# leducthanhig/image-restoration-models

Measured on AMD Instinct MI355X. Metric: images/sec + PSNR, Restormer motion-deblur 1280x720, higher is better.
Workload: dtype f32 (1x1 convs: fp32 emulated by 3 fp16 MFMAs on hi/lo operand splits with fp32 accumulation, error vs float64 at the level of an fp32 chain; everything else exact f32; value_exact_f32: f32 MFMA everywhere); 1 GPU; Restormer motion-deblur (WithBias LN, 26.13M params, synthetic weights seed 42) on 1280x720x3 uint8 GoPro-shaped synthetic frames; 6 tiles 512x512 (overlap 96) per frame; a step = 4 frame(s) per GPU, their 24 tiles in one batched forward; global_batch=4, tile=512, overlap=96, parallelism=per-image shard x1, no data-path collective

## Files before the change

### image-restoration-models_amd/_hip.py

```python
from __future__ import annotations

import ctypes as C
import os

import torch

_HERE = os.path.dirname(os.path.abspath(__file__))
LIB_PATH = os.path.join(_HERE, "libirm_hip.so")

ACT_NONE, ACT_RELU, ACT_GELU, ACT_SILU, ACT_RELU6 = 0, 1, 2, 3, 4
LN_NONE, LN_WITHBIAS, LN_BIASFREE = 0, 1, 2

_P, _L, _I, _F, _D = C.c_void_p, C.c_long, C.c_int, C.c_float, C.c_double

SIGNATURES = {
    "irm_version": [],
    "irm_ln_stats_f32": [_P, _L, _P, _I, _I, _I, _F, _P],
    "irm_gemm1x1_f32": [_P, _L, _P, _L, _P, _L, _P, _L, _P, _P, _P, _P, _I, _I, _I, _I, _I, _I, _I, _I, _P, _F, _P, _P],
    "irm_gemm1x1_f16x3_f32": [_P, _L, _P, _L, _P, _L, _P, _L, _P, _P, _P, _P, _I, _I, _I, _I, _I, _I, _I, _I, _P, _F, _P, _P],
    "irm_ln_split_f16": [_P, _L, _P, _P, _I, _F, _F, _P, _I, _I, _I, _P],
    "irm_ln_gemm_presplit_f16x3_f32": [_P, _P, _L, _P, _P, _I, _F, _F, _P, _L, _P, _F, _I, _I, _I, _I, _I, _P],
    "irm_ln_gemm_presplit_cl_f16x3_f32": [_P, _P, _L, _P, _P, _I, _F, _F, _P, _L, _P, _F, _I, _I, _I, _I, _I, _I, _P],
    "irm_gdfn_tail_f16x3_f32": [_P, _L, _P, _P, _P, _P, _L, _F, _I, _I, _I, _I, _I, _I, _P],
    "irm_gemm_presplit_f16x3_f32": [_P, _P, _P, _L, _P, _F, _I, _I, _I, _I, _I, _I, _I, _I, _P],
# ... 21 lines not shown
    "irm_conv3x3_f16x3_ep_f32": [_P, _F, _P, _L, _P, _L, _P, _L, _P, _I, _I, _I, _I, _I, _I, _F, _I, _I, _I, _I, _I, _I, _P],
    "irm_tile_extract": [_P, _I, _P, _P, _P, _I, _I, _I, _I, _I, _I, _I, _I, _F, _F, _I, _P],
    "irm_chan_stats_f32": [_P, _L, _P, _I, _I, _I, _F, _P],
    "irm_chan_stats_ws_f32": [_P, _L, _P, _P, _L, _I, _I, _I, _F, _P],
    "irm_chan_norm_act_f32": [_P, _L, _P, _P, _P, _P, _L, _P, _L, _I, _I, _I, _I, _P],
    "irm_conv3x3_s2_f32": [_P, _L, _P, _P, _L, _I, _I, _I, _I, _I, _P],
    "irm_dwconv3x3_s2_f32": [_P, _L, _P, _P, _L, _I, _I, _I, _I, _P],
    "irm_upsample_add_f32": [_P, _L, _P, _L, _P, _L, _I, _I, _I, _I, _I, _P],
    "irm_transpose_f32": [_P, _L, _P, _L, _I, _I, _I, _P],
    "irm_selective_scan_f32": [_P, _P, _P, _P, _P, _P, _P, _P, _P, _P, _P, _I, _I, _I, _I, _I, _I, _P],
    "irm_losh_combine_f32": [_P, _P, _P, _P, _P, _P, _P, _P, _L, _P, _L, _I, _I, _I, _I, _F, _P],
    "irm_window_blend": [_P, _P, _P, _P, _I, _P, _P, _I, _I, _I, _I, _I, _I, _I, _I, _I, _I, _F, _F, _P],
    "irm_window_blend_scaled": [_P, _P, _P, _P, _I, _P, _P, _I, _I, _I, _I, _I, _I, _I, _I, _I, _I, _I, _F, _F, _P],
    "irm_frame_metrics": [_P, _P, _I, _I, _I, _I, _I, _D, _P, _P, _P, _L, _P],
    "irm_imresize_bicubic": [_P, _I, _P, _I, _P, _P, _P, _P, _I, _I, _I, _I, _I, _I, _P],
    "irm_frame_metrics_basicsr": [_P, _P, _I, _I, _I, _I, _I, _I, _I, _I, _P, _P, _P, _L, _P],
    "irm_niqe_features": [_P, _I, _I, _I, _I, _I, _I, _I, _P, _P, _P, _L, _P],
    "irm_dihedral_chop_f32": [_P, _P, _P, _L, _I, _I, _I, _I, _I, _I, _I, _P],
    "irm_ensemble_merge_f32": [_P, _P, _P, _L, _I, _I, _I, _I, _I, _I, _P],
}

SIGNATURES_HALF = {
    "irm_conv3x3_h_in_f32": [_P, _P, _L, _P, _L, _P, _I, _I, _I, _I, _I, _I, _P],
    "irm_conv3x3_h_f16": [_P, _F, _P, _L, _P, _L, _P, _L, _P, _I, _I, _I, _I, _I, _I, _I, _I, _P],
    "irm_conv3x3_h_out_f32": [_P, _P, _L, _P, _L, _P, _L, _P, _I, _I, _I, _I, _I, _I, _P],
}

SIGNATURES_FRAMES = {
    "irm_frame_minmax_f32": [_P, _L, _P, _P, _L, _P],
    "irm_tile_extract_f32": [_P, _P, _P, _P, _P, _I, _I, _I, _I, _I, _I, _I, _I, _I, _P],
    "irm_window_blend_f32": [_P, _P, _P, _P, _P, _I, _I, _I, _I, _I, _I, _I, _I, _I, _I, _I, _P],
}

_lib = None


class HipLibraryError(RuntimeError):
    pass


def load():
    global _lib, LIB_PATH
    if _lib is None:
        if os.environ.get("IRM_HIP_LIB"):
            LIB_PATH = os.path.abspath(os.environ["IRM_HIP_LIB"])
        if not os.path.exists(LIB_PATH):
            raise HipLibraryError(
                f"{LIB_PATH} not found: build it with `python -c 'import __graft_entry__ as g; g.build()'` "
                "(make -C image-restoration-models_amd/csrc).  There is no CPU fallback.")
        lib = C.CDLL(LIB_PATH)
        for name, argtypes in {**SIGNATURES, **SIGNATURES_HALF, **SIGNATURES_FRAMES}.items():
            fn = getattr(lib, name)
            fn.argtypes = argtypes
            fn.restype = _I
        _lib = lib
    return _lib


def _stream() -> int:
    return torch.cuda.current_stream().cuda_stream


def ptr(t):
    if t is None:
        return None
    if isinstance(t, int):
        return t
    assert t.is_cuda, "HIP kernels need device tensors"
    return t.data_ptr()


def call(name: str, *args):
    rc = getattr(load(), name)(*args, _stream())
    if rc != 0:
        raise HipLibraryError(f"{name} failed with status {rc} "
                              f"({'invalid arguments' if rc == -1 else 'HIP launch error'})")



def pack_gemm_weight(w: torch.Tensor) -> torch.Tensor:
    w = w.detach().reshape(w.shape[0], -1).float()
    m, k = w.shape
    mt, ks = (m + 15) // 16, 4 * ((k + 15) // 16)
    wpad = torch.zeros(mt * 16, ks * 4, dtype=torch.float32, device=w.device)
# ... 402 lines not shown
```

### image-restoration-models_amd/csrc/fused_qkv_cm.hip

```cpp
#include "irm_common.h"

#define QC_TH 8
#define QC_TW 32
#define QC_PITCH 36
#define QC_SLOTS ((QC_TH + 2) * QC_PITCH)
#define QC_PT 23
#define QC_CS 1728
#define QC_IMG (32 * QC_CS)

struct QcArgs {
    const float* X; long x_bs;
    float* Y; long y_bs;
    const float* rec;
    int C, H, W, S, M;
    int ln_mode; float eps, inv_s1;
    int x_tm, v_tm;
    int tiles_x, tiles, items, gpx;
    const float* gscale;
    float* part;
};
#define QC_NCH 4

__device__ __forceinline__ unsigned qc_row(int c) {
    const int i = c & 15;
    const int rk = i < 4 ? i : i < 12 ? i - 4 : i - 8;
    const int o = (rk >> 1) * 4 + (rk & 1);
    const int fix = (16 - ((c * (QC_CS / 16)) & 15)) & 15;
    return (unsigned)(c * QC_CS + 16 * ((o + fix) & 15));
}

template <int KS, bool GRAM = false>
__global__ __launch_bounds__(512, 2) void qkv_cm_kernel(QcArgs a) {
    static_assert(!GRAM || KS == 2, "GRAM: C = 48");
    constexpr int W1F = KS * 1024, RECF = W1F + 512, RECP = KS * 4 + 2;
    constexpr int SLOT_B = RECF * 4, CF_OFF = W1F * 4;
    constexpr int OSC_OFF = 3 * SLOT_B, MSK_OFF = OSC_OFF + 368 * 4, PL_OFF = MSK_OFF + 368 * 4;
    static_assert(PL_OFF % 16 == 0 && PL_OFF + 2 * QC_IMG <= 160 * 1024, "LDS");
    static_assert(15 * 16 + 368 * 4 <= QC_CS, "row + phase shift inside the row stride");
    extern __shared__ __attribute__((aligned(16))) float smem[];
    irm_lc* lds = (irm_lc*)smem;
    float* slots = smem;

    const int wave = __builtin_amdgcn_readfirstlane((int)threadIdx.x >> 6);
    const long plane = (long)a.H * a.W;
    const int S = a.S;
    const int per = GRAM ? (a.items / QC_NCH + 7) >> 3 : (a.items + 7) >> 3;
    const int xcd = blockIdx.x & 7, pos = blockIdx.x >> 3;
    auto item_of = [&](int round) {
        if constexpr (GRAM) {
            const int i = (round / QC_NCH) * a.gpx + pos;
            return i < per ? (xcd * per + i) * QC_NCH + round % QC_NCH : a.items;
        }
        const int i = round * a.gpx + pos; return i < per ? xcd * per + i : a.items;
    };

    int round = 0;
    int item = item_of(0);
    if (item >= a.items) return;
    float xr[3][KS][8];
    f32x4 gacc[GRAM ? 3 : 1][GRAM ? 3 : 1];
    float gnq[3] = {0.f, 0.f, 0.f}, gnk[3] = {0.f, 0.f, 0.f};
    if constexpr (GRAM) {
#pragma unroll
        for (int x = 0; x < 3; ++x)
#pragma unroll
            for (int y = 0; y < 3; ++y) gacc[x][y] = (f32x4){0.f, 0.f, 0.f, 0.f};
    }
    for (;;) {
        int tid = threadIdx.x;
        asm volatile("" : "+v"(tid));
        const int lane = tid & 63, g = lane >> 4, r = lane & 15;
        const int b = item / a.tiles, tile = item - b * a.tiles;
        const int ty0 = (tile / a.tiles_x) * QC_TH, tx0 = (tile % a.tiles_x) * QC_TW;
        float* Y = a.Y + (long)b * a.y_bs;
        const int nitem = item_of(round + 1);
        const unsigned vw = irm_opaque((unsigned)(lane * 16));

        bool inside[3];
#pragma unroll
        for (int j = 0; j < 3; ++j) {
            const int p = 16 * (wave + 8 * j) + r, ph = p / QC_PITCH, pc = p - ph * QC_PITCH;
            const int gy0 = ty0 - 1 + ph, gx0 = tx0 - 1 + pc;
            inside[j] = p < QC_SLOTS && pc < QC_TW + 2 && gy0 >= 0 && gy0 < a.H && gx0 >= 0 && gx0 < a.W;
        }
        auto load_x = [&](int item) {
            int t2 = threadIdx.x;
            asm volatile("" : "+v"(t2));
            const int r = t2 & 15, g = (t2 & 63) >> 4;
            const int b = item / a.tiles, tile = item - b * a.tiles;
            const int ty0 = (tile / a.tiles_x) * QC_TH, tx0 = (tile % a.tiles_x) * QC_TW;
            const float* X = a.X + (long)b * a.x_bs;
#pragma unroll
        for (int j = 0; j < 3; ++j) {
            const int p = 16 * (wave + 8 * j) + r, ph = p / QC_PITCH, pc = p - ph * QC_PITCH;
            const int gy0 = ty0 - 1 + ph, gx0 = tx0 - 1 + pc;
            const int gy = min(max(gy0, 0), a.H - 1), gx = min(max(gx0, 0), a.W - 1);
            if (a.x_tm) {
                const float* xp = X + (unsigned)((((gy >> 3) * a.tiles_x + (gx >> 5)) * 256 + (gy & 7) * QC_TW + (gx & 31)) * a.C);
#pragma unroll
                for (int ks = 0; ks < KS; ++ks) {
// ... 105 lines not shown
                        acc[j] = __builtin_amdgcn_mfma_f32_16x16x32_f16(xl[j][ks], bh, acc[j], 0, 0, 0);
                        acc[j] = __builtin_amdgcn_mfma_f32_16x16x32_f16(xh[j][ks], bh, acc[j], 0, 0, 0);
                    }
                }
                const float b1 = irm_ld<float>(lds, (unsigned)(r * 4), slot * SLOT_B + CF_OFF + 320 * 4 + hct * 64);
                const unsigned vr = hct ? vrow1 : vrow0;
#pragma unroll
                for (int j = 0; j < 3; ++j) {
                    if (wave + 8 * j < QC_PT) {
                        f32x4 h;
#pragma unroll
                        for (int e = 0; e < 4; ++e) h[e] = fmaf(acc[j][e], osc4[j][e], b1 * msk4[j][e]);
                        irm_st<f32x4>(lds, vr + (unsigned)((16 * (wave + 8 * j) + 4 * g) * 4), PL_OFF + img * QC_IMG, h);
                    }
                }
            }
        };
        auto gemm1 = [&](int slot, int img) { gemm1h(slot, img, 0); gemm1h(slot, img, 1); };
        f32x4 sp0[3], sp1[3];
        irm_v2 sp2[3];
        float stap[10];
        auto st_read = [&](int slot, int img, int hct) {
            const unsigned vr = (hct ? vrow1 : vrow0) + (unsigned)((wave * QC_PITCH + 8 * g) * 4);
            const unsigned vt = (unsigned)((16 * hct + r) * 4);
#pragma unroll
            for (int dy = 0; dy < 3; ++dy) {
                sp0[dy] = irm_ld<f32x4>(lds, vr, PL_OFF + img * QC_IMG + dy * QC_PITCH * 4);
                sp1[dy] = irm_ld<f32x4>(lds, vr, PL_OFF + img * QC_IMG + dy * QC_PITCH * 4 + 16);
                sp2[dy] = irm_ld<irm_v2>(lds, vr, PL_OFF + img * QC_IMG + dy * QC_PITCH * 4 + 32);
            }
#pragma unroll
            for (int t = 0; t < 10; ++t) stap[t] = irm_ld<float>(lds, vt, slot * SLOT_B + CF_OFF + t * 128);
        };
        irm_h8 gqh[GRAM ? 3 : 1], gql[GRAM ? 3 : 1];
        auto st_comp = [&](int st, int hct, auto UC) {
            {
                constexpr int U = decltype(UC)::value;
                const int ch = 32 * st + 16 * hct + r;
                float o[8];
#pragma unroll
                for (int e = 0; e < 8; ++e) o[e] = stap[9];
#pragma unroll
                for (int dy = 0; dy < 3; ++dy) {
                    const float P[10] = {sp0[dy][0], sp0[dy][1], sp0[dy][2], sp0[dy][3], sp1[dy][0], sp1[dy][1], sp1[dy][2], sp1[dy][3],
                                         sp2[dy][0], sp2[dy][1]};
#pragma unroll
                    for (int dx = 0; dx < 3; ++dx) {
                        const float t = stap[dy * 3 + dx];
#pragma unroll
                        for (int e = 0; e < 8; ++e) o[e] = fmaf(t, P[e + dx], o[e]);
                    }
                }
                if constexpr (GRAM && U >= 0 && U < 6) {
                    const float sc = a.gscale[16 * U + r];
                    float nn = 0.f, xs[8];
#pragma unroll
                    for (int e = 0; e < 8; ++e) { nn = fmaf(o[e], o[e], nn); xs[e] = o[e] * sc; }
                    irm_h8 hi, lo;
                    irm_split8(xs, hi, lo);
                    if constexpr (U < 3) {
                        gnq[U] += nn; gqh[U] = hi; gql[U] = lo;
                    } else {
                        gnk[U - 3] += nn;
#pragma unroll
                        for (int x = 0; x < 3; ++x) {
                            f32x4& t = gacc[x][U - 3];
                            t = irm_mfma3_f16(gqh[x], gql[x], hi, lo, t);
                        }
                    }
                    return;
                }
                if (ch >= a.M) return;
                if (ch < 2 * a.C) {
                    float* yt = Y + (long)tile * (2L * a.C * 256) + ch * 256 + wave * QC_TW + 8 * g;
                    *reinterpret_cast<f32x4*>(yt) = (f32x4){o[0], o[1], o[2], o[3]};
                    *reinterpret_cast<f32x4*>(yt + 4) = (f32x4){o[4], o[5], o[6], o[7]};
                } else if (a.v_tm) {
                    float* yt = Y + 2L * a.C * plane + (long)tile * (a.C * 256L) + (wave * QC_TW + 8 * g) * a.C + (ch - 2 * a.C);
#pragma unroll
                    for (int e = 0; e < 8; ++e) yt[e * a.C] = o[e];
                } else {
                    float* yt = Y + (long)ch * plane + (long)(ty0 + wave) * a.W + tx0 + 8 * g;
                    *reinterpret_cast<f32x4*>(yt) = (f32x4){o[0], o[1], o[2], o[3]};
                    *reinterpret_cast<f32x4*>(yt + 4) = (f32x4){o[4], o[5], o[6], o[7]};
                }
            }
        };

        gemm1(0, 0);
        asm volatile("s_waitcnt lgkmcnt(0)" ::: "memory");
        __builtin_amdgcn_s_barrier();
        constexpr std::integral_constant<int, -1> NOU{};
        if constexpr (GRAM) {
            irm_for<5>([&](auto ITC) {
                constexpr int it = decltype(ITC)::value;
                constexpr int s1c = (it + 1) % 3, s3c = it % 3;
                if constexpr (it + 1 < 5) {
                    if constexpr (it + 3 <= 5) irm_dma<RECP>(a.rec + (long)(it + 3) * RECF, slots + s3c * RECF, wave, lane);
                    st_read(s1c, it & 1, 0); gemm1h(s1c, (it + 1) & 1, 0); st_comp(it, 0, std::integral_constant<int, 2 * it>{});
                    st_read(s1c, it & 1, 1); gemm1h(s1c, (it + 1) & 1, 1); st_comp(it, 1, std::integral_constant<int, 2 * it + 1>{});
                    if constexpr (it + 3 <= 5) asm volatile("s_waitcnt vmcnt(0) lgkmcnt(0)" ::: "memory");
                    else asm volatile("s_waitcnt lgkmcnt(0)" ::: "memory");
// ... 4 lines not shown
                    asm volatile("s_waitcnt lgkmcnt(0)" ::: "memory");
                }
                __builtin_amdgcn_s_barrier();
            });
        } else {
        const int it_pf = max(S - 3, 0);
        int s1 = 1, s3 = 0;
        for (int it = 0; it + 1 < S; ++it) {
            const bool dma = it + 3 <= S;
            if (dma) irm_dma<RECP>(a.rec + (long)(it + 3) * RECF, slots + s3 * RECF, wave, lane);
            st_read(s1, it & 1, 0); gemm1h(s1, (it + 1) & 1, 0); st_comp(it, 0, NOU);
            st_read(s1, it & 1, 1); gemm1h(s1, (it + 1) & 1, 1); st_comp(it, 1, NOU);
            if (it <= it_pf) asm volatile("s_waitcnt vmcnt(0) lgkmcnt(0)" ::: "memory");
            else asm volatile("s_waitcnt lgkmcnt(0)" ::: "memory");
            if (PREFETCH && it == it_pf) { load_x(min(nitem, a.items - 1)); __builtin_amdgcn_sched_barrier(0); }
            __builtin_amdgcn_s_barrier();
            s1 = s1 == 2 ? 0 : s1 + 1;
            s3 = s3 == 2 ? 0 : s3 + 1;
        }
        {
            const int it = S - 1;
            if (!PREFETCH || S < 2) {
                load_x(min(nitem, a.items - 1));
                __builtin_amdgcn_sched_barrier(0);
            }
            st_read(s1, it & 1, 0); st_comp(it, 0, NOU);
            st_read(s1, it & 1, 1); st_comp(it, 1, NOU);
            asm volatile("s_waitcnt lgkmcnt(0)" ::: "memory");
            __builtin_amdgcn_s_barrier();
        }
        }
        if constexpr (GRAM) {
            if (round % QC_NCH == QC_NCH - 1) {
                constexpr int REC = 48 * 48 + 96;
#pragma unroll
                for (int t = 0; t < 3; ++t) {
                    gnq[t] += __shfl_xor(gnq[t], 16); gnq[t] += __shfl_xor(gnq[t], 32);
                    gnk[t] += __shfl_xor(gnk[t], 16); gnk[t] += __shfl_xor(gnk[t], 32);
                }
                float* mine = reinterpret_cast<float*>(smem) + PL_OFF / 4 + wave * REC;
                float isk[3];
#pragma unroll
                for (int y = 0; y < 3; ++y) isk[y] = 1.0f / a.gscale[48 + 16 * y + r];
#pragma unroll
                for (int x = 0; x < 3; ++x) {
                    const f32x4 sq4 = *reinterpret_cast<const f32x4*>(a.gscale + 16 * x + 4 * g);
#pragma unroll
                    for (int e = 0; e < 4; ++e) {
                        const float isq = 1.0f / sq4[e];
#pragma unroll
                        for (int y = 0; y < 3; ++y) mine[(16 * x + 4 * g + e) * 48 + 16 * y + r] = gacc[x][y][e] * (isq * isk[y]);
                    }
                    if (g == 0) { mine[48 * 48 + 16 * x + r] = gnq[x]; mine[48 * 48 + 48 + 16 * x + r] = gnk[x]; }
                }
                __syncthreads();
                const float* all = reinterpret_cast<const float*>(smem) + PL_OFF / 4;
                float* out = a.part + ((long)b * (a.tiles / QC_NCH) + tile / QC_NCH) * REC;
                for (int e = threadIdx.x; e < REC; e += 512) {
                    float sum = all[e];
#pragma unroll
                    for (int w = 1; w < 8; ++w) sum += all[w * REC + e];
                    out[e] = sum;
                }
#pragma unroll
                for (int x = 0; x < 3; ++x) {
                    gnq[x] = 0.f; gnk[x] = 0.f;
#pragma unroll
                    for (int y = 0; y < 3; ++y) gacc[x][y] = (f32x4){0.f, 0.f, 0.f, 0.f};
                }
            }
        }
        if (nitem >= a.items) break;
        item = nitem;
        ++round;
    }
}

template <int KS, bool GRAM = false>
static int qc_launch(QcArgs a, int B, hipStream_t stream) {
    const size_t lds = (size_t)3 * (KS * 1024 + 512) * 4 + 2 * 368 * 4 + 2 * QC_IMG;
    IRM_ALLOW_BIG_LDS((&qkv_cm_kernel<KS, GRAM>));
    int dev = 0, n = 0;
    if (hipGetDevice(&dev) != hipSuccess ||
        hipDeviceGetAttribute(&n, hipDeviceAttributeMultiprocessorCount, dev) != hipSuccess || n <= 0) return IRM_ELAUNCH;
    a.tiles_x = a.W / QC_TW;
    a.tiles = a.tiles_x * (a.H / QC_TH);
    a.items = B * a.tiles;
    const int per = GRAM ? (a.items / QC_NCH + 7) >> 3 : (a.items + 7) >> 3;
    a.gpx = (n + 7) / 8;
    if (a.gpx > per) a.gpx = per;
    hipLaunchKernelGGL((qkv_cm_kernel<KS, GRAM>), dim3(a.gpx * 8), dim3(512), lds, stream, a);
    return irm_launch_status();
}

extern "C" int irm_qkv_gram_cm_f16x3_f32(const float* rec, const float* x, long x_bs, float* y, long y_bs, const float* gscale,
                                         float* part, int ln_mode, float eps, float inv_s1, int B, int C, int H, int W, int x_tm,
                                         int v_tm, hipStream_t stream) {
    if (!rec || !x || !y || !gscale || !part || x == y || B <= 0 || H <= 0 || W <= 0) return IRM_EINVAL;
    if (C != 48 || (H & 7) || (W & 31) || ((H / 8) * (W / 32)) % QC_NCH || (long)3 * C * H * W >= (1L << 30)) return IRM_EINVAL;
    if (ln_mode != IRM_LN_WITHBIAS && ln_mode != IRM_LN_BIASFREE) return IRM_EINVAL;
    if ((x_bs & 3) || (y_bs & 3) || !irm_aligned16(x) || !irm_aligned16(y) || !irm_aligned16(rec) || !irm_aligned16(gscale)) return IRM_EINVAL;
    QcArgs a;
// ... 24 lines not shown
```

### image-restoration-models_amd/ops.py

```python
from __future__ import annotations

import os

import torch

from . import _hip
from ._hip import ACT_GELU, ACT_NONE, ACT_RELU, ACT_RELU6, ACT_SILU, LN_BIASFREE, LN_NONE, LN_WITHBIAS


class KernelTimer:

    def __init__(self, detail=False, only=None):
        self.records = []
        self.detail = detail
        self.only = None if only is None else frozenset(only)
        self._chain = {}
        self._done = {}
        self._since = 0

    def _fold(self, k, e0, e1, fl, by):
        d = self._done.setdefault(k, dict(launches=0, ms=0.0, flops=0.0, bytes=0.0))
        d["launches"] += 1
        d["ms"] += e0.elapsed_time(e1)
        d["flops"] += fl
# ... 285 lines not shown
    rec = c * c + 2 * c
    if c in (48, 96) and N % 64 == 0:
        slots, best = 2 * 256, None
        for chunk in range(128, 4096 + 1, 64):
            nchunk = -(-N // chunk)
            cost = -(-(B * heads * nchunk) // slots) * (chunk + 192)
            if best is None or cost < best[0]:
                best = (cost, chunk, nchunk)
        return best[1], best[2], rec
    nsub = (c // (16 * sb)) ** 2
    chunk = -(-(N * B * heads * nsub) // (4 * target_blocks()))
    chunk = min(max(-(-chunk // 64) * 64, 256), 4096)
    return chunk, -(-N // chunk), rec


QKV_GRAM_NCH = 4


def can_qkv_gram(C: int, heads: int, H: int, W: int) -> bool:
    return C == 48 and heads == 1 and H % 8 == 0 and W % 32 == 0 and ((H // 8) * (W // 32)) % QKV_GRAM_NCH == 0


def qkv_gram_cm(pk, x, y, gram_scale, part, C: int, *, ln_mode, eps: float = 1e-5, x_tm: bool = False, v_tm: bool = False) -> int:
    _chk(x, "x"), _chk(y, "y")
    B, _, H, W = x.shape
    assert can_qkv_gram(C, 1, H, W) and y.shape[1] == 3 * C and gram_scale.numel() == 2 * C
    rec, inv_s1 = pk
    N = H * W
    nchunk = (H // 8) * (W // 32) // QKV_GRAM_NCH
    assert part.numel() >= B * nchunk * (C * C + 2 * C)
    _launch("qkv_dw_fused", B * N * (2.0 * 3 * C * C + 18.0 * 3 * C + 2.0 * C * C), 4.0 * B * N * 2 * C, "irm_qkv_gram_cm_f16x3_f32",
            _hip.ptr(rec), _hip.ptr(x), _bs(x), _hip.ptr(y), _bs(y), _hip.ptr(gram_scale), _hip.ptr(part), int(ln_mode),
            float(eps), float(inv_s1), B, C, H, W, int(x_tm), int(v_tm), tag=f"C{C} {H}x{W} B{B} gram")
    return nchunk


def mdta_fold(qkv, part, gsum, temperature, wout, mfold, C: int, heads: int, attn=None, split: bool = False,
              gram_scale=None, frag: bool = False, tm: bool = False, nchunk_ready: int | None = None):
    _chk(qkv, "qkv")
    B, _, H, W = qkv.shape
    N = H * W
    chunk, nchunk, rec = mdta_plan(B, C, heads, N)
    if nchunk_ready is not None:
        nchunk = nchunk_ready
    assert part.numel() >= B * heads * nchunk * rec and gsum.numel() >= B * heads * rec
    c = C // heads
    assert not tm or (c in (48, 96) and N % 256 == 0), "tile-major q, k: the LDS-DMA ring passes only"
    if nchunk_ready is not None:
        pass
    elif gram_scale is not None and c in (48, 96) and N % 64 == 0:
        assert gram_scale.numel() == 2 * C and gram_scale.is_contiguous()
        _launch("mdta_gram_f16x3", 2.0 * B * heads * c * c * N, 8.0 * B * C * N,
                "irm_mdta_gram_tm_f16x3_f32" if tm else "irm_mdta_gram_f16x3_f32", _hip.ptr(qkv),
                _bs(qkv), _hip.ptr(gram_scale), _hip.ptr(part), B, C, heads, N, chunk,
                tag=f"C{C} h{heads} N{N} B{B} chunk{chunk}")
    else:
        _launch("mdta_gram", 2.0 * B * heads * c * c * N, 8.0 * B * C * N, "irm_mdta_gram_tm_f32" if tm else "irm_mdta_gram_f32",
                _hip.ptr(qkv), _bs(qkv), _hip.ptr(part), B, C, heads, N, chunk, tag=f"C{C} h{heads} N{N} B{B} chunk{chunk}")
    _launch("mdta_finalize", 2.0 * B * C * C * c, 4.0 * B * (heads * nchunk * rec + C * C),
            "irm_mdta_finalize_frag_f16x3_f32" if frag else "irm_mdta_finalize_f16x3_f32" if split else "irm_mdta_finalize_f32",
            _hip.ptr(part), _hip.ptr(gsum), _hip.ptr(temperature), _hip.ptr(wout), _hip.ptr(mfold), _hip.ptr(attn),
            B, C, heads, nchunk, tag=f"C{C} h{heads} nchunk{nchunk} B{B}")


def can_fuse_stats(M: int) -> bool:
    mt = (M + 15) // 16
# ... 154 lines not shown
```

### image-restoration-models_amd/restormer/restormer.py

```python
from __future__ import annotations

import os

import torch
import torch.nn as nn

from .. import _hip, ops

SYNTH_RULES = (
    (r"^output\.weight$", "gain", 0.02),
    (r"^skip_conv\.weight$", "gain", 0.5),
)


def _hidden(dim, factor):
    return int(dim * factor)


class _Norm(nn.Module):

    def __init__(self, dim, kind):
        super().__init__()
        self.body = nn.Module()
        self.body.weight = nn.Parameter(torch.ones(dim))
# ... 119 lines not shown
                a, ff = m.attn, m.ffn
                pk[name] = dict(
                    qkv=_hip.pack_gemm_weight(a.qkv.weight), qkv_b=f32(a.qkv.bias),
                    qkv_dw=f32(a.qkv_dwconv.weight.reshape(-1, 9)), qkv_dw_b=f32(a.qkv_dwconv.bias),
                    wout=f32(a.project_out.weight.reshape(m.dim, m.dim)), wout_b=f32(a.project_out.bias),
                    temp=f32(a.temperature.reshape(-1)),
                    pin=_hip.pack_gemm_weight(ff.project_in.weight), pin_b=f32(ff.project_in.bias),
                    ffn_dw=f32(ff.dwconv.weight.reshape(-1, 9)), ffn_dw_b=f32(ff.dwconv.bias),
                    pout=_hip.pack_gemm_weight(ff.project_out.weight), pout_b=f32(ff.project_out.bias),
                    n1w=f32(m.norm1.w), n1b=f32(m.norm1.b), n2w=f32(m.norm2.w), n2b=f32(m.norm2.b))
                if self._split:
                    if _hip.split_is_safe(a.qkv.weight, m.norm1.w, m.norm1.b):
                        pk[name]["qkv_s"] = _hip.pack_gemm_weight_split(a.qkv.weight)
                    if _hip.split_is_safe(ff.project_in.weight, m.norm2.w, m.norm2.b):
                        pk[name]["pin_s"] = _hip.pack_gemm_weight_split(ff.project_in.weight)
                    if _hip.split_is_safe(ff.project_out.weight):
                        pk[name]["pout_s"] = _hip.pack_gemm_weight_split(ff.project_out.weight)
                    pk[name]["mfold_split"] = _hip.split_is_safe(a.project_out.weight)
                    if m.dim == 192:
                        hp = 64 * -(-ff.hidden // 64)
                        frag, s_w, bp = _hip.pack_pin_padded(ff.project_in.weight, ff.project_in.bias, hp)
                        s_x = _hip.ln_split_scale(m.norm2.w, m.norm2.b, m.dim, m.norm2.mode == ops.LN_WITHBIAS)
                        pk[name]["pin_cl"] = (frag, 1.0 / (s_w * s_x), s_x, bp, hp)
                        pk[name]["tail"] = _hip.pack_gdfn_tail(ff.dwconv.weight, ff.dwconv.bias, ff.project_out.weight)
                    if m.dim in (192, 384):
                        for slot, conv, nrm in (("qkv_ps", a.qkv, m.norm1), ("pin_ps", ff.project_in, m.norm2)):
                            frag, s_w = _hip.pack_gemm_weight_presplit(conv.weight)
                            s_x = _hip.ln_split_scale(nrm.w, nrm.b, m.dim, nrm.mode == ops.LN_WITHBIAS)
                            pk[name][slot] = (frag, 1.0 / (s_w * s_x), s_x)
                    gs = _hip.gram_scales(a.qkv.weight, a.qkv.bias, a.qkv_dwconv.weight, a.qkv_dwconv.bias, m.norm1.w,
                                          m.norm1.b, m.norm1.mode == ops.LN_WITHBIAS)
                    if gs is not None:
                        pk[name]["gram_s"] = gs.to(a.qkv.weight.device)
                if self._split and ops.can_fuse_gdfn(m.dim, 4):
                    pk[name].update(
                        qkv_f=_hip.pack_qkv_fused(a.qkv.weight, a.qkv.bias, a.qkv_dwconv.weight, a.qkv_dwconv.bias,
                                                  m.norm1.w, m.norm1.b),
                        gdfn_f=_hip.pack_gdfn_fused(ff.project_in.weight, ff.project_in.bias, ff.dwconv.weight,
                                                    ff.dwconv.bias, ff.project_out.weight, m.norm2.w, m.norm2.b))
                    if pk[name]["mfold_split"] and m.dim % 16 == 0:
                        pk[name]["gdfn_fa"] = _hip.pack_gdfn_fused(
                            ff.project_in.weight, ff.project_in.bias, ff.dwconv.weight, ff.dwconv.bias,
                            ff.project_out.weight, m.norm2.w, m.norm2.b, kperm=True)
                if ops.can_fuse_dw(m.dim, 4):
                    c, dw, dwb = m.dim, a.qkv_dwconv.weight.reshape(-1, 9), a.qkv_dwconv.bias
                    pk[name].update(
                        v_dwp=_hip.pack_dw_table(dw[2 * c:], None if dwb is None else dwb[2 * c:], c, False),
                        ffn_dwp=_hip.pack_dw_table(ff.dwconv.weight, ff.dwconv.bias, ff.hidden, True))
        for name in ("down1_2", "down2_3", "down3_4", "up4_3", "up3_2", "up2_1"):
            pk[name] = _hip.pack_conv3x3(getattr(self, name).body[0].weight)
        pk["patch_embed"] = _hip.pack_conv3x3(self.patch_embed.proj.weight)
        pk["patch_embed_b"] = f32(self.patch_embed.proj.bias)
        pk["output"] = _hip.pack_conv3x3(self.output.weight)
        pk["output_b"] = f32(self.output.bias)
        for name in ("reduce_chan_level3", "reduce_chan_level2") + (("skip_conv",) if self.dual_pixel_task else ()):
            pk[name] = _hip.pack_gemm_weight(getattr(self, name).weight)
            pk[name + "_b"] = f32(getattr(self, name).bias)
            if self._split and name != "skip_conv" and _hip.split_is_safe(getattr(self, name).weight):
                pk[name + "_s"] = _hip.pack_gemm_weight_split(getattr(self, name).weight)
        self._packed, self._packed_key = pk, key
        return pk

    @property
    def _ws(self):
        return self._ws_by_stream.setdefault(torch.cuda.current_stream().cuda_stream if torch.cuda.is_available()
                                             else 0, {})
# ... 15 lines not shown
        return t

    def release_workspace(self):
        self._ws_by_stream.clear()

    def _block(self, blk: TransformerBlock, w: dict, x: torch.Tensor, have_stats: bool = False,
               want_stats: bool = True) -> bool:
        B, C, H, W = x.shape
        N = H * W
        dev = x.device
        heads = blk.attn.num_heads
        hid = blk.ffn.hidden
        fuse = ops.can_fuse_stats(C)
        stats = self._buf("stats", B * 2 * N, dev)
        big_a = self._buf("scratch_a", B * max(3 * C, 2 * hid) * N, dev)
        big_b = self._buf("scratch_b", B * max(3 * C, hid) * N, dev)
        qkv = big_a[:B * 3 * C * N].view(B, 3 * C, H, W)
        qkv2 = big_b[:B * 3 * C * N].view(B, 3 * C, H, W)
        split = self._split and N % 4 == 0
        s_qkv, s_pin, s_pout = split and "qkv_s" in w, split and "pin_s" in w, split and "pout_s" in w
        s_fold = split and w.get("mfold_split", False)
        presplit = split and "qkv_ps" in w and ops.can_presplit(C, N)
        if presplit:
            xs = self._buf("xsplit", B * C * N, dev)
            frag, out_scale, s_x = w["qkv_ps"]
            ops.ln_gemm_presplit(frag, x, qkv, 3 * C, C, w["n1w"], w["n1b"], blk.norm1.mode, s_x, out_scale=out_scale,
                                 bias=w["qkv_b"], xs=xs)
        else:
            if not have_stats:
                ops.ln_stats(x, stats)
            ops.gemm1x1(w["qkv_s" if s_qkv else "qkv"], x, qkv, 3 * C, C, bias=w["qkv_b"], stats=stats, lnw=w["n1w"],
                        lnb=w["n1b"], ln_mode=blk.norm1.mode, split=s_qkv)
        fuse_dw = "v_dwp" in w and ops.can_fuse_dw(C, W)
        if fuse_dw:
            ops.dwconv3x3(qkv[:, :2 * C], w["qkv_dw"], qkv2[:, :2 * C],
                          bias=None if w["qkv_dw_b"] is None else w["qkv_dw_b"][:2 * C])
        else:
            ops.dwconv3x3(qkv, w["qkv_dw"], qkv2, bias=w["qkv_dw_b"])
        _, nchunk, rec = ops.mdta_plan(B, C, heads, N)
        part = self._buf("gram_part", B * heads * nchunk * rec, dev)
        gsum = self._buf("gram_sum", B * heads * rec, dev)
        mfold_n = ops.mfold_numel(C)
        mfold = self._zeros(("mfold", C, B), B * mfold_n, dev)
        ops.mdta_fold(qkv2, part, gsum, w["temp"], w["wout"], mfold, C, heads, split=s_fold,
                      gram_scale=w.get("gram_s") if split else None)
        if fuse_dw:
            ops.dwgemm(mfold, w["v_dwp"], qkv[:, 2 * C:], x, C, C, gate=False, res=x, bias=w["wout_b"],
                       w_bs=mfold_n, stats_out=stats if fuse else None, split=s_fold)
        else:
            ops.gemm1x1(mfold, qkv2[:, 2 * C:], x, C, C, res=x, bias=w["wout_b"], w_bs=mfold_n,
                        stats_out=stats if fuse else None, split=s_fold)
        if split and "tail" in w and ops.can_gdfn_tail(C, H, W):
            frag, out_scale, s_x, bp, hp = w["pin_cl"]
            h_cl = self._buf("h_cl", B * 2 * hp * N, dev)
            ops.ln_gemm_presplit_cl(frag, x, h_cl, 2 * hp, C, w["n2w"], w["n2b"], blk.norm2.mode, s_x, out_scale=out_scale, bias=bp)
            ops.gdfn_tail(w["tail"], h_cl, x, C, hid, hp, bias=w["pout_b"])
            return False
        h = big_a[:B * 2 * hid * N].view(B, 2 * hid, H, W)
        g = big_b[:B * hid * N].view(B, hid, H, W)
        if presplit:
            frag, out_scale, s_x = w["pin_ps"]
            ops.ln_gemm_presplit(frag, x, h, 2 * hid, C, w["n2w"], w["n2b"], blk.norm2.mode, s_x, out_scale=out_scale,
                                 bias=w["pin_b"], xs=xs)
        else:
            if not fuse:
                ops.ln_stats(x, stats)
            ops.gemm1x1(w["pin_s" if s_pin else "pin"], x, h, 2 * hid, C, bias=w["pin_b"], stats=stats, lnw=w["n2w"],
                        lnb=w["n2b"], ln_mode=blk.norm2.mode, split=s_pin)
        emit = fuse and want_stats
        if fuse_dw:
            ops.dwgemm(w["pout_s" if s_pout else "pout"], w["ffn_dwp"], h, x, C, hid, gate=True, res=x,
                       bias=w["pout_b"], stats_out=stats if emit else None, split=s_pout)
        else:
            ops.dwconv3x3_gate(h, w["ffn_dw"], g, bias=w["ffn_dw_b"])
            ops.gemm1x1(w["pout_s" if s_pout else "pout"], g, x, C, hid, res=x, bias=w["pout_b"],
                        stats_out=stats if emit else None, split=s_pout)
        return emit

# ... 127 lines not shown
```

### include/irm_hip.h

```cpp
#ifndef IRM_HIP_H
#define IRM_HIP_H

#ifdef __cplusplus
extern "C" {
#endif

typedef struct ihipStream_t* irm_stream_t;

#define IRM_OK 0
#define IRM_EINVAL (-1)
#define IRM_ELAUNCH (-2)

#define IRM_ACT_NONE 0
#define IRM_ACT_RELU 1
#define IRM_ACT_GELU 2
#define IRM_ACT_SILU 3

#define IRM_LN_NONE 0
#define IRM_LN_WITHBIAS 1
#define IRM_LN_BIASFREE 2

int irm_version(void);

int irm_ln_stats_f32(const float* x, long x_bs, float* stats, int B, int C, int N, float eps,
// ... 124 lines not shown
int irm_chan_stats_f32(const float* x, long x_bs, float* stats, int B, int C, int N, float eps, irm_stream_t stream);
int irm_chan_stats_ws_f32(const float* x, long x_bs, float* stats, float* ws, long ws_floats, int B, int C, int N,
                          float eps, irm_stream_t stream);
int irm_chan_norm_act_f32(const float* x, long x_bs, const float* stats, const float* w, const float* b,
                          const float* res, long r_bs, float* y, long y_bs, int B, int C, int N, int act,
                          irm_stream_t stream);
int irm_conv3x3_s2_f32(const float* x, long x_bs, const float* w, float* y, long y_bs, int B, int Ci, int Co, int H,
                       int W, irm_stream_t stream);
int irm_dwconv3x3_s2_f32(const float* x, long x_bs, const float* w, float* y, long y_bs, int B, int C, int H, int W,
                         irm_stream_t stream);
int irm_upsample_add_f32(const float* src, long s_bs, const float* add, long a_bs, float* out, long o_bs, int B, int C,
                         int Hs, int Ws, int scale, irm_stream_t stream);

int irm_dihedral_chop_f32(const float* src, const int* table, float* dst, long dst_pixels, int B, int C, int H, int W,
                          int P, int max_ph, int max_pw, irm_stream_t stream);
int irm_ensemble_merge_f32(const float* pred, const int* table, float* out, long pred_pixels, int B, int Co, int H,
                           int W, int P, int scale, irm_stream_t stream);

int irm_transpose_f32(const float* in, long in_bs, float* out, long out_bs, int B, int R, int C,
                      irm_stream_t stream);

int irm_selective_scan_f32(const float* xT, const float* pT, const int* ids, const float* dtw, const float* dtb,
                           const float* A, const float* Dskip, float* yT, float* state, float* sdt, float* ysum,
                           int B, int L, int D, int N, int R, int chunk, irm_stream_t stream);

int irm_losh_combine_f32(float* ysum, const float* gw, const float* gb, float* gate, const float* yT,
                         const float* nw, const float* nb, const float* z, long z_bs, float* out, long out_bs,
                         int B, int L, int D, int nchunk, float eps, irm_stream_t stream);

#include "irm_hip_half.h"

#include "irm_hip_frames.h"

#ifdef __cplusplus
}
#endif
#endif
```

Before: 21.79 images/s.

## Fuse q/k depthwise 3x3 conv with Gram accumulation for C=192/384 attention

```diff
diff --git a/image-restoration-models_amd/_hip.py b/image-restoration-models_amd/_hip.py
--- a/image-restoration-models_amd/_hip.py
+++ b/image-restoration-models_amd/_hip.py
@@ -77,6 +77,10 @@
     "irm_window_blend_f32": [_P, _P, _P, _P, _P, _I, _I, _I, _I, _I, _I, _I, _I, _I, _I, _I, _P],
 }
 
+SIGNATURES_GRAM = {
+    "irm_dw_gram_cm_f16x3_f32": [_P, _L, _P, _P, _P, _P, _I, _I, _I, _I, _I, _P],
+}
+
 _lib = None
 
 
@@ -94,7 +98,7 @@
                 f"{LIB_PATH} not found: build it with `python -c 'import __graft_entry__ as g; g.build()'` "
                 "(make -C image-restoration-models_amd/csrc).  There is no CPU fallback.")
         lib = C.CDLL(LIB_PATH)
-        for name, argtypes in {**SIGNATURES, **SIGNATURES_HALF, **SIGNATURES_FRAMES}.items():
+        for name, argtypes in {**SIGNATURES, **SIGNATURES_HALF, **SIGNATURES_FRAMES, **SIGNATURES_GRAM}.items():
             fn = getattr(lib, name)
             fn.argtypes = argtypes
             fn.restype = _I
diff --git a/image-restoration-models_amd/csrc/dw_gram.hip b/image-restoration-models_amd/csrc/dw_gram.hip
--- /dev/null
+++ b/image-restoration-models_amd/csrc/dw_gram.hip
@@ -0,0 +1,200 @@
+#include "irm_common.h"
+#include "gram_cm.h"
+
+struct DgArgs {
+    const float* qkv; long bs;
+    const float* taps;
+    const float* bias;
+    const float* gscale;
+    float* part;
+    int C, heads, H, W;
+    int tiles_x, cpi, units, gpx;
+};
+
+constexpr int DG_PIECES = 32 * (QC_TH + 2) * 9;
+constexpr int DG_PF = (DG_PIECES + 511) / 512;
+constexpr int DG_TAP_OFF = 2 * QC_IMG;
+constexpr int DG_LDS = DG_TAP_OFF + 10 * 96 * 4;
+typedef float dg_f4u __attribute__((ext_vector_type(4), aligned(4)));
+
+__global__ __launch_bounds__(512) void dw_gram_kernel(DgArgs a) {
+    static_assert(8 * QC_REC * 4 <= 2 * QC_IMG, "the chunk-end reduction fits in the image area");
+    static_assert(15 * 16 + QC_SLOTS * 4 <= QC_CS, "row + phase shift inside the row stride");
+    extern __shared__ __attribute__((aligned(16))) float smem[];
+    irm_lc* lds = (irm_lc*)smem;
+
+    const int wave = __builtin_amdgcn_readfirstlane((int)threadIdx.x >> 6);
+    const int tid = threadIdx.x, lane = tid & 63, g = lane >> 4, r = lane & 15;
+    const unsigned plane = (unsigned)(a.H * a.W);
+    const int per = (a.units + 7) >> 3;
+    const int xcd = blockIdx.x & 7, pos = blockIdx.x >> 3;
+    auto unit_of = [&](int k) {
+        const int i = k * a.gpx + pos, u = xcd * per + i;
+        return i < per && u < a.units ? u : a.units;
+    };
+    int k = 0, unit = unit_of(0);
+    if (unit >= a.units) return;
+
+    unsigned pdst[DG_PF], pdesc[DG_PF];
+#pragma unroll
+    for (int j = 0; j < DG_PF; ++j) {
+        const int e = min(tid + 512 * j, DG_PIECES - 1);
+        const int ch = e / 90, row = (e % 90) / 9, pc = e % 9;
+        pdesc[j] = (unsigned)(ch | row << 8 | pc << 16);
+        pdst[j] = qc_row(ch) + (unsigned)((row * QC_PITCH + 4 * pc) * 4);
+    }
+
+    f32x4 pv[DG_PF];
+    unsigned prowok = 0;
+    bool pleft = false, pright = false;
+    auto request = [&](int u, int t, int s) {
+        const int bh = u / a.cpi, tile = (u - bh * a.cpi) * QC_NCH + t;
+        const int b = bh / a.heads, head = bh - b * a.heads;
+        const int ty0 = (tile / a.tiles_x) * QC_TH, tx0 = (tile % a.tiles_x) * QC_TW;
+        const float* src = a.qkv + (long)b * a.bs;
+        pleft = tx0 == 0;
+        pright = tx0 + QC_TW == a.W;
+        prowok = 0;
+#pragma unroll
+        for (int j = 0; j < DG_PF; ++j) {
+            const unsigned d = irm_opaque(pdesc[j]);
+            const int pc = (int)(d >> 16);
+            const int cc = 32 * s + (int)(d & 255);
+            const int ch = head * 48 + (cc < 48 ? cc : a.C + cc - 48);
+            const int gy = ty0 - 1 + (int)((d >> 8) & 255);
+            if (gy >= 0 && gy < a.H) prowok |= 1u << j;
+            const int gx = tx0 - 1 + 4 * pc + ((pc == 0 && pleft) ? 1 : 0) - ((pc == 8 && pright) ? 3 : 0);
+            const unsigned off = (unsigned)ch * plane + (unsigned)(min(max(gy, 0), a.H - 1) * a.W + gx);
+            pv[j] = *reinterpret_cast<const dg_f4u*>(src + off);
+        }
+    };
+    auto park = [&](unsigned img) {
+#pragma unroll
+        for (int j = 0; j < DG_PF; ++j) {
+            f32x4 v = pv[j];
+            const int pc = (int)(irm_opaque(pdesc[j]) >> 16);
+            if (pc == 0 && pleft) v = (f32x4){0.f, v[0], v[1], v[2]};
+            if (pc == 8 && pright) v = (f32x4){v[3], 0.f, 0.f, 0.f};
+            if (!((prowok >> j) & 1)) v = (f32x4){0.f, 0.f, 0.f, 0.f};
+            irm_st<f32x4>(lds, pdst[j] + img, 0, v);
+        }
+    };
+    auto put_taps = [&](int u) {
+        const int bh = u / a.cpi, head = bh % a.heads;
+#pragma unroll
+        for (int j = 0; j < 2; ++j) {
+            const int e = tid + 512 * j;
+            if (e < 960) {
+                const int t = e / 96, cc = e - 96 * t;
+                const int ch = head * 48 + (cc < 48 ? cc : a.C + cc - 48);
+                const float v = t < 9 ? a.taps[ch * 9 + t] : (a.bias ? a.bias[ch] : 0.f);
+                irm_st<float>(lds, (unsigned)(DG_TAP_OFF + e * 4), 0, v);
+            }
+        }
+    };
+
+    QcGram gram;
+    qc_gram_clear(gram);
+    const unsigned vrow0 = qc_row(r) + (unsigned)((wave * QC_PITCH + 8 * g) * 4);
+    const unsigned vrow1 = qc_row(16 + r) + (unsigned)((wave * QC_PITCH + 8 * g) * 4);
+    const unsigned vtap = irm_opaque((unsigned)(DG_TAP_OFF + r * 4));
+
+    put_taps(unit);
+    request(unit, 0, 0);
+    park(0);
+    __syncthreads();
+    for (;;) {
+        const int bh = unit / a.cpi;
+        const int head = bh % a.heads;
+        const float* sq = a.gscale + head * 48;
+        const float* sk = a.gscale + a.C + head * 48;
+        const int nunit = unit_of(k + 1);
+        float gsc[6];
+#pragma unroll
+        for (int u = 0; u < 6; ++u) gsc[u] = (u < 3 ? sq : sk)[16 * (u % 3) + r];
+        irm_h8 gqh[QC_NCH][3], gql[QC_NCH][3];
+        irm_for<3>([&](auto SC) {
+            irm_for<QC_NCH>([&](auto TC) {
+                constexpr int s = decltype(SC)::value, t = decltype(TC)::value;
+                constexpr bool last = s == 2 && t + 1 == QC_NCH;
+                constexpr int IMG = ((s * QC_NCH + t) & 1) * QC_IMG, NIMG = QC_IMG - IMG;
+                static_assert((3 * QC_NCH) % 2 == 0, "a chunk starts in image 0");
+                const bool more = !last || nunit < a.units;
+                if (more) {
+                    if constexpr (t + 1 < QC_NCH) request(unit, t + 1, s);
+                    else if constexpr (s < 2) request(unit, 0, s + 1);
+                    else request(nunit, 0, 0);
+                }
+                __builtin_amdgcn_sched_barrier(0);
+                irm_for<2>([&](auto HC) {
+                    constexpr int hct = decltype(HC)::value, U = 2 * s + hct;
+                    const unsigned vr = hct ? vrow1 : vrow0;
+                    f32x4 sp0[3], sp1[3];
+                    irm_v2 sp2[3];
+                    float stap[10];
+#pragma unroll
+                    for (int dy = 0; dy < 3; ++dy) {
+                        sp0[dy] = irm_ld<f32x4>(lds, vr, IMG + dy * QC_PITCH * 4);
+                        sp1[dy] = irm_ld<f32x4>(lds, vr, IMG + dy * QC_PITCH * 4 + 16);
+                        sp2[dy] = irm_ld<irm_v2>(lds, vr, IMG + dy * QC_PITCH * 4 + 32);
+                    }
+#pragma unroll
+                    for (int tp = 0; tp < 10; ++tp) stap[tp] = irm_ld<float>(lds, vtap, (tp * 96 + 16 * U) * 4);
+                    float o[8];
+#pragma unroll
+                    for (int e = 0; e < 8; ++e) o[e] = stap[9];
+#pragma unroll
+                    for (int dy = 0; dy < 3; ++dy) {
+                        const float P[10] = {sp0[dy][0], sp0[dy][1], sp0[dy][2], sp0[dy][3], sp1[dy][0], sp1[dy][1], sp1[dy][2],
+                                             sp1[dy][3], sp2[dy][0], sp2[dy][1]};
+#pragma unroll
+                        for (int dx = 0; dx < 3; ++dx) {
+                            const float tp = stap[dy * 3 + dx];
+#pragma unroll
+                            for (int e = 0; e < 8; ++e) o[e] = fmaf(tp, P[e + dx], o[e]);
+                        }
+                    }
+                    qc_gram_unit<U>(gram, gqh[t], gql[t], o, gsc[U]);
+                    irm_tie(gram.nq[0], gram.nq[1], gram.nq[2], gram.nk[0], gram.nk[1], gram.nk[2]);
+                    __builtin_amdgcn_sched_barrier(0);
+                });
+                if constexpr (last) {
+                    __syncthreads();
+                    qc_gram_flush(gram, smem, sq, sk, a.part, (long)unit, wave, g, r);
+                    __syncthreads();
+                    if (more) put_taps(nunit);
+                }
+                if (more) park((unsigned)NIMG);
+                __syncthreads();
+            });
+        });
+        if (nunit >= a.units) break;
+        unit = nunit;
+        ++k;
+    }
+}
+
+extern "C" int irm_dw_gram_cm_f16x3_f32(const float* qkv, long bs, const float* taps, const float* bias, const float* gscale,
+                                        float* part, int B, int C, int heads, int H, int W, hipStream_t stream) {
+    if (!qkv || !taps || !gscale || !part || B <= 0 || C <= 0 || heads <= 0 || H <= 0 || W <= 0) return IRM_EINVAL;
+    if (C % heads || C / heads != 48 || (H & 7) || (W & 31)) return IRM_EINVAL;
+    const long tiles = (long)(H / QC_TH) * (W / QC_TW);
+    if (tiles % QC_NCH || (long)3 * C * H * W >= (1L << 30) || bs < (long)2 * C * H * W) return IRM_EINVAL;
+    if ((bs & 3) || !irm_aligned16(qkv) || !irm_aligned16(gscale) || (reinterpret_cast<uintptr_t>(part) & 3) ||
+        (reinterpret_cast<uintptr_t>(taps) & 3) || (reinterpret_cast<uintptr_t>(bias) & 3)) return IRM_EINVAL;
+    const long units = (long)B * heads * (tiles / QC_NCH);
+    if (units >= (1L << 28)) return IRM_EINVAL;
+    IRM_ALLOW_BIG_LDS((&dw_gram_kernel));
+    int dev = 0, n = 0;
+    if (hipGetDevice(&dev) != hipSuccess ||
+        hipDeviceGetAttribute(&n, hipDeviceAttributeMultiprocessorCount, dev) != hipSuccess || n <= 0) return IRM_ELAUNCH;
+    DgArgs a;
+    a.qkv = qkv; a.bs = bs; a.taps = taps; a.bias = bias; a.gscale = gscale; a.part = part;
+    a.C = C; a.heads = heads; a.H = H; a.W = W;
+    a.tiles_x = W / QC_TW; a.cpi = (int)(tiles / QC_NCH); a.units = (int)units;
+    const int per = (a.units + 7) >> 3;
+    a.gpx = (n + 7) / 8;
+    if (a.gpx > per) a.gpx = per;
+    hipLaunchKernelGGL(dw_gram_kernel, dim3(a.gpx * 8), dim3(512), DG_LDS, stream, a);
+    return irm_launch_status();
+}
diff --git a/image-restoration-models_amd/csrc/fused_qkv_cm.hip b/image-restoration-models_amd/csrc/fused_qkv_cm.hip
--- a/image-restoration-models_amd/csrc/fused_qkv_cm.hip
+++ b/image-restoration-models_amd/csrc/fused_qkv_cm.hip
@@ -1,12 +1,5 @@
 #include "irm_common.h"
-
-#define QC_TH 8
-#define QC_TW 32
-#define QC_PITCH 36
-#define QC_SLOTS ((QC_TH + 2) * QC_PITCH)
-#define QC_PT 23
-#define QC_CS 1728
-#define QC_IMG (32 * QC_CS)
+#include "gram_cm.h"
 
 struct QcArgs {
     const float* X; long x_bs;
@@ -19,15 +12,6 @@
     const float* gscale;
     float* part;
 };
-#define QC_NCH 4
-
-__device__ __forceinline__ unsigned qc_row(int c) {
-    const int i = c & 15;
-    const int rk = i < 4 ? i : i < 12 ? i - 4 : i - 8;
-    const int o = (rk >> 1) * 4 + (rk & 1);
-    const int fix = (16 - ((c * (QC_CS / 16)) & 15)) & 15;
-    return (unsigned)(c * QC_CS + 16 * ((o + fix) & 15));
-}
 
 template <int KS, bool GRAM = false>
 __global__ __launch_bounds__(512, 2) void qkv_cm_kernel(QcArgs a) {
@@ -58,14 +42,8 @@
     int item = item_of(0);
     if (item >= a.items) return;
     float xr[3][KS][8];
-    f32x4 gacc[GRAM ? 3 : 1][GRAM ? 3 : 1];
-    float gnq[3] = {0.f, 0.f, 0.f}, gnk[3] = {0.f, 0.f, 0.f};
-    if constexpr (GRAM) {
-#pragma unroll
-        for (int x = 0; x < 3; ++x)
-#pragma unroll
-            for (int y = 0; y < 3; ++y) gacc[x][y] = (f32x4){0.f, 0.f, 0.f, 0.f};
-    }
+    QcGram gram;
+    if constexpr (GRAM) qc_gram_clear(gram);
     for (;;) {
         int tid = threadIdx.x;
         asm volatile("" : "+v"(tid));
@@ -237,7 +215,7 @@
 #pragma unroll
             for (int t = 0; t < 10; ++t) stap[t] = irm_ld<float>(lds, vt, slot * SLOT_B + CF_OFF + t * 128);
         };
-        irm_h8 gqh[GRAM ? 3 : 1], gql[GRAM ? 3 : 1];
+        irm_h8 gqh[3], gql[3];
         auto st_comp = [&](int st, int hct, auto UC) {
             {
                 constexpr int U = decltype(UC)::value;
@@ -257,22 +235,7 @@
                     }
                 }
                 if constexpr (GRAM && U >= 0 && U < 6) {
-                    const float sc = a.gscale[16 * U + r];
-                    float nn = 0.f, xs[8];
-#pragma unroll
-                    for (int e = 0; e < 8; ++e) { nn = fmaf(o[e], o[e], nn); xs[e] = o[e] * sc; }
-                    irm_h8 hi, lo;
-                    irm_split8(xs, hi, lo);
-                    if constexpr (U < 3) {
-                        gnq[U] += nn; gqh[U] = hi; gql[U] = lo;
-                    } else {
-                        gnk[U - 3] += nn;
-#pragma unroll
-                        for (int x = 0; x < 3; ++x) {
-                            f32x4& t = gacc[x][U - 3];
-                            t = irm_mfma3_f16(gqh[x], gql[x], hi, lo, t);
-                        }
-                    }
+                    qc_gram_unit<U>(gram, gqh, gql, o, a.gscale[16 * U + r]);
                     return;
                 }
                 if (ch >= a.M) return;
@@ -343,42 +306,8 @@
         }
         if constexpr (GRAM) {
             if (round % QC_NCH == QC_NCH - 1) {
-                constexpr int REC = 48 * 48 + 96;
-#pragma unroll
-                for (int t = 0; t < 3; ++t) {
-                    gnq[t] += __shfl_xor(gnq[t], 16); gnq[t] += __shfl_xor(gnq[t], 32);
-                    gnk[t] += __shfl_xor(gnk[t], 16); gnk[t] += __shfl_xor(gnk[t], 32);
-                }
-                float* mine = reinterpret_cast<float*>(smem) + PL_OFF / 4 + wave * REC;
-                float isk[3];
-#pragma unroll
-                for (int y = 0; y < 3; ++y) isk[y] = 1.0f / a.gscale[48 + 16 * y + r];
-#pragma unroll
-                for (int x = 0; x < 3; ++x) {
-                    const f32x4 sq4 = *reinterpret_cast<const f32x4*>(a.gscale + 16 * x + 4 * g);
-#pragma unroll
-                    for (int e = 0; e < 4; ++e) {
-                        const float isq = 1.0f / sq4[e];
-#pragma unroll
-                        for (int y = 0; y < 3; ++y) mine[(16 * x + 4 * g + e) * 48 + 16 * y + r] = gacc[x][y][e] * (isq * isk[y]);
-                    }
-                    if (g == 0) { mine[48 * 48 + 16 * x + r] = gnq[x]; mine[48 * 48 + 48 + 16 * x + r] = gnk[x]; }
-                }
-                __syncthreads();
-                const float* all = reinterpret_cast<const float*>(smem) + PL_OFF / 4;
-                float* out = a.part + ((long)b * (a.tiles / QC_NCH) + tile / QC_NCH) * REC;
-                for (int e = threadIdx.x; e < REC; e += 512) {
-                    float sum = all[e];
-#pragma unroll
-                    for (int w = 1; w < 8; ++w) sum += all[w * REC + e];
-                    out[e] = sum;
-                }
-#pragma unroll
-                for (int x = 0; x < 3; ++x) {
-                    gnq[x] = 0.f; gnk[x] = 0.f;
-#pragma unroll
-                    for (int y = 0; y < 3; ++y) gacc[x][y] = (f32x4){0.f, 0.f, 0.f, 0.f};
-                }
+                qc_gram_flush(gram, reinterpret_cast<float*>(smem) + PL_OFF / 4, a.gscale, a.gscale + 48,
+                              a.part, (long)b * (a.tiles / QC_NCH) + tile / QC_NCH, wave, g, r);
             }
         }
         if (nitem >= a.items) break;
diff --git a/image-restoration-models_amd/csrc/gram_cm.h b/image-restoration-models_amd/csrc/gram_cm.h
--- /dev/null
+++ b/image-restoration-models_amd/csrc/gram_cm.h
@@ -0,0 +1,87 @@
+#pragma once
+#include "irm_common.h"
+
+constexpr int QC_TH = 8, QC_TW = 32;
+constexpr int QC_PITCH = 36;
+constexpr int QC_SLOTS = (QC_TH + 2) * QC_PITCH;
+constexpr int QC_PT = 23;
+constexpr int QC_CS = 1728;
+constexpr int QC_IMG = 32 * QC_CS;
+constexpr int QC_NCH = 4;
+constexpr int QC_REC = 48 * 48 + 96;
+
+__device__ __forceinline__ unsigned qc_row(int c) {
+    const int i = c & 15;
+    const int rk = i < 4 ? i : i < 12 ? i - 4 : i - 8;
+    const int o = (rk >> 1) * 4 + (rk & 1);
+    const int fix = (16 - ((c * (QC_CS / 16)) & 15)) & 15;
+    return (unsigned)(c * QC_CS + 16 * ((o + fix) & 15));
+}
+
+struct QcGram {
+    f32x4 acc[3][3];
+    float nq[3], nk[3];
+};
+
+__device__ __forceinline__ void qc_gram_clear(QcGram& s) {
+#pragma unroll
+    for (int x = 0; x < 3; ++x) {
+        s.nq[x] = 0.f; s.nk[x] = 0.f;
+#pragma unroll
+        for (int y = 0; y < 3; ++y) s.acc[x][y] = (f32x4){0.f, 0.f, 0.f, 0.f};
+    }
+}
+
+template <int U>
+__device__ __forceinline__ void qc_gram_unit(QcGram& s, irm_h8 (&qh)[3], irm_h8 (&ql)[3], const float (&o)[8], float sc) {
+    static_assert(U >= 0 && U < 6, "three q tiles, three k tiles");
+    float nn = 0.f, xs[8];
+#pragma unroll
+    for (int e = 0; e < 8; ++e) { nn = fmaf(o[e], o[e], nn); xs[e] = o[e] * sc; }
+    irm_h8 hi, lo;
+    irm_split8(xs, hi, lo);
+    if constexpr (U < 3) {
+        s.nq[U] += nn; qh[U] = hi; ql[U] = lo;
+    } else {
+        s.nk[U - 3] += nn;
+#pragma unroll
+        for (int x = 0; x < 3; ++x) {
+            f32x4& t = s.acc[x][U - 3];
+            t = irm_mfma3_f16(qh[x], ql[x], hi, lo, t);
+        }
+    }
+}
+
+__device__ __forceinline__ void qc_gram_flush(QcGram& s, float* scratch, const float* sq, const float* sk, float* part, long rec,
+                                              int wave, int g, int r) {
+#pragma unroll
+    for (int t = 0; t < 3; ++t) {
+        s.nq[t] += __shfl_xor(s.nq[t], 16); s.nq[t] += __shfl_xor(s.nq[t], 32);
+        s.nk[t] += __shfl_xor(s.nk[t], 16); s.nk[t] += __shfl_xor(s.nk[t], 32);
+    }
+    float* mine = scratch + wave * QC_REC;
+    float isk[3];
+#pragma unroll
+    for (int y = 0; y < 3; ++y) isk[y] = 1.0f / sk[16 * y + r];
+#pragma unroll
+    for (int x = 0; x < 3; ++x) {
+        const f32x4 sq4 = *reinterpret_cast<const f32x4*>(sq + 16 * x + 4 * g);
+#pragma unroll
+        for (int e = 0; e < 4; ++e) {
+            const float isq = 1.0f / sq4[e];
+#pragma unroll
+            for (int y = 0; y < 3; ++y) mine[(16 * x + 4 * g + e) * 48 + 16 * y + r] = s.acc[x][y][e] * (isq * isk[y]);
+        }
+        if (g == 0) { mine[48 * 48 + 16 * x + r] = s.nq[x]; mine[48 * 48 + 48 + 16 * x + r] = s.nk[x]; }
+    }
+    __syncthreads();
+    const float* all = scratch;
+    float* out = part + rec * QC_REC;
+    for (int e = threadIdx.x; e < QC_REC; e += 512) {
+        float sum = all[e];
+#pragma unroll
+        for (int w = 1; w < 8; ++w) sum += all[w * QC_REC + e];
+        out[e] = sum;
+    }
+    qc_gram_clear(s);
+}
diff --git a/image-restoration-models_amd/ops.py b/image-restoration-models_amd/ops.py
--- a/image-restoration-models_amd/ops.py
+++ b/image-restoration-models_amd/ops.py
@@ -341,6 +341,25 @@
     _launch("qkv_dw_fused", B * N * (2.0 * 3 * C * C + 18.0 * 3 * C + 2.0 * C * C), 4.0 * B * N * 2 * C, "irm_qkv_gram_cm_f16x3_f32",
             _hip.ptr(rec), _hip.ptr(x), _bs(x), _hip.ptr(y), _bs(y), _hip.ptr(gram_scale), _hip.ptr(part), int(ln_mode),
             float(eps), float(inv_s1), B, C, H, W, int(x_tm), int(v_tm), tag=f"C{C} {H}x{W} B{B} gram")
+    return nchunk
+
+
+def can_dw_gram(C: int, heads: int, H: int, W: int) -> bool:
+    return (C in (192, 384) and C == 48 * heads and H % 8 == 0 and W % 32 == 0
+            and ((H // 8) * (W // 32)) % QKV_GRAM_NCH == 0 and 3 * C * H * W < 1 << 30)
+
+
+def dw_gram(qkv, w9, gram_scale, part, C: int, heads: int, *, bias=None) -> int:
+    _chk(qkv, "qkv")
+    B, _, H, W = qkv.shape
+    N = H * W
+    assert can_dw_gram(C, heads, H, W) and qkv.shape[1] >= 2 * C and gram_scale.numel() == 2 * C and gram_scale.is_contiguous()
+    assert w9.shape == (2 * C, 9) and w9.is_contiguous() and (bias is None or (bias.numel() == 2 * C and bias.is_contiguous()))
+    nchunk = (H // 8) * (W // 32) // QKV_GRAM_NCH
+    assert part.numel() >= B * heads * nchunk * (48 * 48 + 96)
+    _launch("dw_gram", B * N * (18.0 * 2 * C + 2.0 * 48 * C), 4.0 * B * N * 2 * C, "irm_dw_gram_cm_f16x3_f32", _hip.ptr(qkv),
+            _bs(qkv), _hip.ptr(w9), _hip.ptr(bias), _hip.ptr(gram_scale), _hip.ptr(part), B, C, heads, H, W,
+            tag=f"C{C} h{heads} {H}x{W} B{B}")
     return nchunk
 
 
diff --git a/image-restoration-models_amd/restormer/restormer.py b/image-restoration-models_amd/restormer/restormer.py
--- a/image-restoration-models_amd/restormer/restormer.py
+++ b/image-restoration-models_amd/restormer/restormer.py
@@ -175,6 +175,9 @@
                                           m.norm1.b, m.norm1.mode == ops.LN_WITHBIAS)
                     if gs is not None:
                         pk[name]["gram_s"] = gs.to(a.qkv.weight.device)
+                        if m.dim in (192, 384):
+                            c2, dwb = 2 * m.dim, a.qkv_dwconv.bias
+                            pk[name]["qk_dw"] = (f32(a.qkv_dwconv.weight.reshape(-1, 9)[:c2]), None if dwb is None else f32(dwb[:c2]))
                 if self._split and ops.can_fuse_gdfn(m.dim, 4):
                     pk[name].update(
                         qkv_f=_hip.pack_qkv_fused(a.qkv.weight, a.qkv.bias, a.qkv_dwconv.weight, a.qkv_dwconv.bias,
@@ -256,18 +259,26 @@
             ops.gemm1x1(w["qkv_s" if s_qkv else "qkv"], x, qkv, 3 * C, C, bias=w["qkv_b"], stats=stats, lnw=w["n1w"],
                         lnb=w["n1b"], ln_mode=blk.norm1.mode, split=s_qkv)
         fuse_dw = "v_dwp" in w and ops.can_fuse_dw(C, W)
-        if fuse_dw:
+        gram_dw = split and "gram_s" in w and "qk_dw" in w and ops.can_dw_gram(C, heads, H, W)
+        _, nchunk, rec = ops.mdta_plan(B, C, heads, N)
+        if gram_dw:
+            nchunk = (H // 8) * (W // 32) // ops.QKV_GRAM_NCH
+        part = self._buf("gram_part", B * heads * nchunk * rec, dev)
+        nready = None
+        if gram_dw:
+            nready = ops.dw_gram(qkv, w["qk_dw"][0], w["gram_s"], part, C, heads, bias=w["qk_dw"][1])
+            ops.dwconv3x3(qkv[:, 2 * C:], w["qkv_dw"][2 * C:], qkv2[:, 2 * C:],
+                          bias=None if w["qkv_dw_b"] is None else w["qkv_dw_b"][2 * C:])
+        elif fuse_dw:
             ops.dwconv3x3(qkv[:, :2 * C], w["qkv_dw"], qkv2[:, :2 * C],
                           bias=None if w["qkv_dw_b"] is None else w["qkv_dw_b"][:2 * C])
         else:
             ops.dwconv3x3(qkv, w["qkv_dw"], qkv2, bias=w["qkv_dw_b"])
-        _, nchunk, rec = ops.mdta_plan(B, C, heads, N)
-        part = self._buf("gram_part", B * heads * nchunk * rec, dev)
         gsum = self._buf("gram_sum", B * heads * rec, dev)
         mfold_n = ops.mfold_numel(C)
         mfold = self._zeros(("mfold", C, B), B * mfold_n, dev)
         ops.mdta_fold(qkv2, part, gsum, w["temp"], w["wout"], mfold, C, heads, split=s_fold,
-                      gram_scale=w.get("gram_s") if split else None)
+                      gram_scale=w.get("gram_s") if split else None, nchunk_ready=nready)
         if fuse_dw:
             ops.dwgemm(mfold, w["v_dwp"], qkv[:, 2 * C:], x, C, C, gate=False, res=x, bias=w["wout_b"],
                        w_bs=mfold_n, stats_out=stats if fuse else None, split=s_fold)
diff --git a/include/irm_hip.h b/include/irm_hip.h
--- a/include/irm_hip.h
+++ b/include/irm_hip.h
@@ -180,6 +180,8 @@
 
 #include "irm_hip_frames.h"
 
+#include "irm_hip_gram.h"
+
 #ifdef __cplusplus
 }
 #endif
diff --git a/include/irm_hip_gram.h b/include/irm_hip_gram.h
--- /dev/null
+++ b/include/irm_hip_gram.h
@@ -0,0 +1,4 @@
+#pragma once
+
+int irm_dw_gram_cm_f16x3_f32(const float* qkv, long bs, const float* taps, const float* bias, const float* gscale, float* part,
+                             int B, int C, int heads, int H, int W, irm_stream_t stream);
```

Result: faster. 22.06 images/s, median of 6 (+1.2%).
